# yhinai/EIG-KL-Algorithm

Measured on AMD Instinct MI355X. Metric: wall-clock to final cut (s) + cut size, ibm18.hgr; SpMV GB/s vs HBM peak, lower is better.
Workload: dtype f64 (Lanczos) + f32 (KL gains, bit-exact with cKL)

## Files before the change

eig-kl-algorithm_amd/csrc/ctx_lanczos.cpp:

```cpp
#include "ctx.hpp"

#ifndef EK_UPD_RED_MAX_NRB
#define EK_UPD_RED_MAX_NRB 256
#endif

using namespace ek::rt;

extern "C" {

void ek_lanczos_default_opts(ek_lanczos_opts* o) {
    if (!o) return;
    o->ncv = 0;
    o->maxit = 1000;
    o->tol = 1e-10;
    o->deflate = 1;
    o->time_spmv = 0;
    o->reorth = 3;
    o->check_every = 8;
    o->basis32 = 1;
    o->alpha_last = 0;
    o->keep_min = -1;
    o->reorth_thresh = 0.0;
}

// ... 236 lines not shown
        ek::dev::ProLaunch pl;
        if (inl) {
            pl.wpart = c->wpart.as<double>();
            pl.alpha = c->alpha.as<double>();
            pl.offd = c->offd.as<double>();
            pl.omega = c->omega.as<double>();
            pl.st = c->prost.as<ek::dev::ProState>();
            pl.flags = c->pflags.as<int>();
            pl.pub = pro_pub();
            pl.a3 = a3;
            pl.seg0 = seg0;
            pl.m = m;
            pl.thresh = pro_thresh;
            pl.eps1 = pro_eps1;
            pl.cgw = pro_cgw;
            static const int tickets = env_flag("EK_PRO_TICKETS", false) ? 2 : env_flag("EK_PRO_TICKETS", true) ? 1 : 0;
            if (tickets) pl.tix = pro_pub() + size_t(ek::dev::PRO_PUB_WORDS) * ek::dev::PRO_PUB_STRIDE;
            if (tickets == 1) {
                pl.cap = ek::dev::gemvt_pro_capacity(nt, c->nrb_spmv > 12 * 256, pro_merge, pro_merge && b32,
                                                     c->num_cu);
                const int ncg_max = (m + has_u0 + ek::dev::GT_COLS - 1) / ek::dev::GT_COLS;
                auto grid = [&](int cg) { return ek::dev::gemvt_pro_grid(nrb, std::min(ncg_max, cg), ldv, pro_merge); };
                int cg = pl.cgw;
                while (!pro_cgw_env && cg > 1 && grid(cg) > pl.cap) --cg;
                if (!pro_cgw_env && cg > 0 && grid(cg) <= pl.cap) pl.cgw = cg;
            }
            pl.rev = env_set("EK_DISPATCH_REVERSE") ? 1 : 0;
            if (pro_merge) {
                pl.merged = 1;
                pl.npart = c->npart.as<double>();
                pl.V32 = V32();
                pl.fb = b32 ? c->fbk.as<unsigned>() : nullptr;
            }
        }
        const bool mrg = inl && pro_merge;
        for (int i = k; i < kend; ++i) {
            ek::dev::StepFin fin;
            if (i > seg0) {
                fin.npart = c->npart.as<double>();
                fin.nb = nub;
                fin.fn2_out = fn2 + i;
                fin.h2 = c->h2.as<double>();
                fin.step = i - 1;
                fin.alpha = c->alpha.as<double>();
                fin.offd = c->offd.as<double>();
                fin.a3 = a3;
                fin.fn2_i = fn2 + i - 1;
                fin.bov_i = bov + i - 1;
// ... 902 lines not shown
```

eig-kl-algorithm_amd/csrc/ek_internal.hpp:

```cpp
#pragma once

#include <cstdint>
#include <cstdio>
#include <cstring>
#include <functional>
#include <memory>
#include <utility>
#include <string>
#include <type_traits>
#include <vector>

#include "../../include/eigkl.h"

namespace ek {
void set_error(const char* fmt, ...) __attribute__((format(printf, 1, 2)));
struct Error {
    int code;
};
[[noreturn]] void fail(int code, const char* fmt, ...) __attribute__((format(printf, 2, 3)));
int guard_exceptions();

int host_threads();
struct ThreadCap {
    explicit ThreadCap(int cap);
// ... 317 lines not shown
              int i, int seg0, int m, double thresh, double eps1);
constexpr int PRO_PUB = 8;
constexpr int PRO_PUB_STRIDE = 64;
constexpr int PRO_PUB_WORDS = PRO_PUB + 1;
struct ProLaunch {
    const double* wpart = nullptr;
    const double* alpha = nullptr;
    const double* offd = nullptr;
    double* omega = nullptr;
    ProState* st = nullptr;
    int* flags = nullptr;
    unsigned* pub = nullptr;
    double* a3 = nullptr;
    double* npart = nullptr;
    const float* V32 = nullptr;
    unsigned* fb = nullptr;
    int merged = 0;
    int cgw = 0;
    int seg0 = 0, m = 0;
    double thresh = 0.0, eps1 = 0.0;
    unsigned* tix = nullptr;
    int rev = 0;
    int cap = 0;
};
int gemvt_pro_capacity(bool nt, bool wide, bool merged, bool b32u, int num_cu);
int gemvt_pro_grid(int nrb, int ncgl, int ldv, bool merged);
void finalize_step(hipStream_t s, const double* npart, int nb, double* fn2_out, const double* h1,
                   const double* h2, int step, double* alpha, double* offd, const double* a3 = nullptr,
                   const double* fn2_i = nullptr, const double* bov_i = nullptr);
void three_term(hipStream_t s, int ldv, const double* apart, int nparts, double* alpha_io, const double* w,
                const double* vi, const double* vim1, const double* fn2_i, const double* bov_i, double* fp,
                float* v32col = nullptr);
void gemm_vq(hipStream_t s, int ldv, const double* V, int m, const double* Q, int kk, double* out,
             float* out32 = nullptr);
void inject_random(hipStream_t s, double* f, int ldv, long long row0, long long nrows, unsigned long long st0);
void zero_pad_rows(hipStream_t s, double* V, int ldv, int nreal, int ncols);
size_t split_tmp_bytes(int n);
void fiedler_scale(hipStream_t s, const double* x, double sgn, int n, double* out);
void split_select(hipStream_t s, void* tmp, const double* v, int n, unsigned k0, unsigned k1,
                  unsigned long long* keys_out);
double key_value(unsigned long long key);
void split_partition(hipStream_t s, void* tmp, const double* v, int n, double med, int32_t* order0, int32_t* order1,
                     uint32_t* plist, uint8_t* side, unsigned* n0_out);
void axpby_norm(hipStream_t s, int ldv, double* f, double sigma, const double* x, double hk, double* npart);
void scale_sub_mean(hipStream_t s, int ldv, double* x, int nreal, const double* mean_sum, double inv_n);
void sum_partial(hipStream_t s, int ldv, const double* x, int nreal, double* npart, int squares);
void resid_partial(hipStream_t s, int ldv, const double* w, const double* x, double lambda, int nreal, double* part);
void start_vector(hipStream_t s, int ldv, long long row0, int nreal, double* x);

// ... 195 lines not shown
```

eig-kl-algorithm_amd/csrc/kernels_lanczos.hip:

```cpp
#include <hip/hip_runtime.h>

#include <cstdio>
#include <cstdlib>

#include "ek_device.hpp"
#include "ek_internal.hpp"

#ifndef EK_UPD_UB
#define EK_UPD_UB 8
#endif

namespace ek {
namespace dev {

#ifdef EK_PRO_STAMPS
constexpr int PRO_STAMP_LO = 20, PRO_STAMP_NS = 80, PRO_STAMP_WG = 2048, PRO_STAMP_W = 6;
__device__ unsigned long long g_pro_stamps[size_t(PRO_STAMP_NS) * PRO_STAMP_WG * PRO_STAMP_W];
__device__ __forceinline__ void pro_stamp(int step, int slot, unsigned long long val) {
    const int k = step - PRO_STAMP_LO;
    if (threadIdx.x == 0 && k >= 0 && k < PRO_STAMP_NS && int(blockIdx.x) < PRO_STAMP_WG)
        g_pro_stamps[(size_t(k) * PRO_STAMP_WG + blockIdx.x) * PRO_STAMP_W + slot] = val;
}
#define PRO_STAMP(slot) pro_stamp(ncols - 1, (slot), __builtin_amdgcn_s_memrealtime())
#define PRO_ROLE(r) pro_stamp(ncols - 1, 0, (r))
#define PRO_DECISION(v) pro_stamp(ncols - 1, 5, (v))
#else
#define PRO_STAMP(slot) ((void)0)
#define PRO_ROLE(r) ((void)0)
#define PRO_DECISION(v) ((void)0)
#endif

#ifndef EK_PRO_CG0_FIRST
#define EK_PRO_CG0_FIRST 1
#endif
#ifndef EK_PRO_NORM_DIRECT
#define EK_PRO_NORM_DIRECT 1
#endif
__host__ __device__ constexpr int pro_slots(int nrb) { return EK_PRO_CG0_FIRST ? (nrb + 7) / 8 * 8 : nrb; }

__device__ __forceinline__ double wave_sum(double v) {
#pragma unroll
    for (int o = 32; o > 0; o >>= 1) v += __shfl_xor(v, o, 64);
    return v;
}

__device__ __forceinline__ double strided_sum256(const double* __restrict__ x, int n) {
    constexpr int SB = 16;
    double s = 0.0;
    if (n <= 0) return s;
    for (int i0 = threadIdx.x; i0 < n; i0 += SB * 256) {
        double v[SB];
#pragma unroll
        for (int u = 0; u < SB; ++u) v[u] = x[min(i0 + u * 256, n - 1)];
#pragma unroll
        for (int u = 0; u < SB; ++u) s += i0 + u * 256 < n ? v[u] : 0.0;
    }
    return s;
}

__device__ __forceinline__ void strided_sum256x2(const double* __restrict__ x, const double* __restrict__ y, int n,
                                                 double& sx, double& sy) {
// ... 149 lines not shown
    __syncthreads();
    double mx = fabs(nv);
#pragma unroll
    for (int o = 32; o > 0; o >>= 1) mx = fmax(mx, __shfl_xor(mx, o, 64));
    if ((t & 63) == 0) mx4[t >> 6] = mx;
    __syncthreads();
    const double mxa = fmax(fmax(mx4[0], mx4[1]), fmax(mx4[2], mx4[3]));
    const bool d = forced || !(mxa <= thresh);
    if (t < i) onew[t] = d ? eps1 : nv;
    if (t == i) onew[i] = eps1;
    if (t == 255) onew[U] = d ? eps1 : nv;
    if (i == seg0) {
        if (t < i) ocur[t] = eps1;
        if (t == 255) ocur[U] = eps1;
    }
    if (t == 0) {
        flags[i] = d ? 1 : 0;
        st->force = (d && !s_pair) ? 1 : 0;
        if (d) st->projected += 1;
    }
    return d;
}

__device__ __forceinline__ void gemvt_skip_tail(int ncols, int has_u0, int nrb, int rbk, int t,
                                                double* __restrict__ part, const double* nred,
                                                unsigned* __restrict__ gctr, double* __restrict__ h_out,
                                                double* __restrict__ fn2_fast, bool zero_h = true,
                                                unsigned* __restrict__ done = nullptr) {
    const int tot = ncols + has_u0, i = ncols - 1;
    __syncthreads();
    const double nb = (nred[0] + nred[1]) + (nred[2] + nred[3]);
    if (!h_out) {
        if (t == 0) part[size_t(tot) * nrb + rbk] = nb;
        if (t == 1) part[size_t(i) * nrb + rbk] = 0.0;
        if (t == 2 && i > 0) part[size_t(i - 1) * nrb + rbk] = 0.0;
        return;
    }
    __shared__ int s_last;
    if (t == 0) {
        st_sc1(part + size_t(tot) * nrb + rbk, nb);
        asm volatile("s_waitcnt vmcnt(0)" ::: "memory");
        const int g = rbk % GT_SUB;
        const unsigned gsize = unsigned((nrb - g + GT_SUB - 1) / GT_SUB), ngroups = unsigned(nrb < GT_SUB ? nrb : GT_SUB);
        int last = 0;
        if (__hip_atomic_fetch_add(gctr + g * 64, 1u, EK_HANDOFF_ORDER, __HIP_MEMORY_SCOPE_AGENT) == gsize - 1u)
            last = __hip_atomic_fetch_add(gctr + GT_SUB * 64, 1u, EK_HANDOFF_ORDER, __HIP_MEMORY_SCOPE_AGENT) ==
                   ngroups - 1u;
        s_last = last;
    }
    __syncthreads();
    if (!s_last) return;
    if (zero_h)
        for (int j = t; j < tot; j += 256) h_out[j] = 0.0;
    if (t < CS_LANES) {
        const double* pc = part + size_t(tot) * nrb;
        constexpr int CB = 32;
        double a = 0.0;
        for (int b0 = t; b0 < nrb; b0 += CS_LANES * CB) {
            double va[CB];
#pragma unroll
            for (int u = 0; u < CB; ++u) va[u] = ld_sc1(pc + min(b0 + CS_LANES * u, nrb - 1));
#pragma unroll
            for (int u = 0; u < CB; ++u) a += b0 + CS_LANES * u < nrb ? va[u] : 0.0;
        }
#pragma unroll
        for (int o = 1; o < CS_LANES; o <<= 1) a += __shfl_xor(a, o, 64);
        if (t == 0) {
            if (done) {
                st_sc1(h_out + tot, a);
                if (fn2_fast) st_sc1(fn2_fast, a);
                asm volatile("s_waitcnt vmcnt(0)" ::: "memory");
                __hip_atomic_fetch_add(done, 1u, __ATOMIC_RELAXED, __HIP_MEMORY_SCOPE_AGENT);
            } else {
                h_out[tot] = a;
                if (fn2_fast) *fn2_fast = a;
            }
        }
    }
    if (t < GT_SUB + 1) gctr[t * 64] = 0u;
}

__device__ __forceinline__ bool pro_aborted(int* err) {
    return __hip_atomic_load(err, __ATOMIC_RELAXED, __HIP_MEMORY_SCOPE_AGENT) != 0;
}
__device__ __forceinline__ int pro_poll(const unsigned* pub, int* err) {
    unsigned v = 0u;
    for (int it = 0; it < (1 << 22); ++it) {
        v = __hip_atomic_load(pub, __ATOMIC_RELAXED, __HIP_MEMORY_SCOPE_AGENT);
        if (v != 0u) break;
        if ((it & 255) == 255 && pro_aborted(err)) break;
        __builtin_amdgcn_s_sleep(8);
    }
    if (v == 0u) atomicAdd(err, 1);
    return v != 0u ? int(v) : 2;
}
__device__ __forceinline__ int pro_wait(const unsigned* ctr, unsigned target, int* err) {
    for (int it = 0; it < (1 << 22); ++it) {
        if (__hip_atomic_load(ctr, __ATOMIC_RELAXED, __HIP_MEMORY_SCOPE_AGENT) >= target) return 1;
        if ((it & 255) == 255 && pro_aborted(err)) break;
        __builtin_amdgcn_s_sleep(4);
    }
    atomicAdd(err, 1);
    return 0;
}

struct UpdTT {
    const double* w = nullptr;
    const double* vi = nullptr;
    const double* vim1 = nullptr;
    const double* fn2_i = nullptr;
    const double* bov_i = nullptr;
    const double* apart = nullptr;
    int nparts = 0;
    int* err = nullptr;
};
template <bool RED, bool B32, bool NT, bool MRG>
__device__ __forceinline__ void update_body(int blk, int ldv, const double* __restrict__ V, int ncols, int has_u0,
                                            double u0val, int nreal, const double* __restrict__ h,
                                            const double* __restrict__ src, double* __restrict__ dst,
                                            double* __restrict__ npart, const double* __restrict__ part, int nrb,
                                            double* __restrict__ h_out, const float* __restrict__ V32,
                                            unsigned* __restrict__ fb, double* __restrict__ fn2_fast,
                                            const unsigned* __restrict__ done, unsigned done_target, UpdTT tt);

template <bool TT, bool NT, int APE, bool PROI, bool MRG = false, bool B32U = false>
__device__ __forceinline__ void gemvt_body(int ldv, int nrb, const double* __restrict__ V, int ncols,
                                               int has_u0, double u0val, int nreal, const double* __restrict__ w,
                                               double* __restrict__ part, const double* __restrict__ alpha,
                                               const double* __restrict__ vi, const double* __restrict__ vim1,
                                               const double* __restrict__ fn2_i, const double* __restrict__ bov_i,
                                               double* __restrict__ fp, int nrm, float* __restrict__ v32col,
                                               const double* __restrict__ apart, int nparts,
                                               double* __restrict__ alpha_pub, unsigned* __restrict__ gctr,
                                               double* __restrict__ h_out, const int* __restrict__ flag,
                                               double* __restrict__ fn2_fast, ProLaunch pl) {
#pragma clang fp contract(off)
    __shared__ double red[4][GT_COLS];
    __shared__ double nred[4];
    __shared__ double lds4[4];
    __shared__ double s_alpha;
    const int t = threadIdx.x;
    const int ncg = (ncols + has_u0 + GT_COLS - 1) / GT_COLS;
    const int ncgl = PROI && pl.cgw > 0 ? min(ncg, pl.cgw) : ncg;
    int nwg = int(gridDim.x), orig = int(blockIdx.x);
    if constexpr (PROI) {
        if (pl.rev) orig = nwg - 1 - orig;
        if (pl.tix) {
            __shared__ int s_orig;
            if (t == 0) {
                const unsigned x = unsigned(orig) & 7u, cnt = (unsigned(nwg) - x + 7u) >> 3;
                unsigned* q = pl.tix + PRO_PUB_STRIDE * x;
                const unsigned j = __hip_atomic_fetch_add(q, 1u, __ATOMIC_RELAXED, __HIP_MEMORY_SCOPE_AGENT);
                if (j == cnt - 1u) __hip_atomic_store(q, 0u, __ATOMIC_RELAXED, __HIP_MEMORY_SCOPE_AGENT);
                s_orig = int(x + 8u * j);
            }
            __syncthreads();
            orig = s_orig;
        }
    }
    if constexpr (PROI) PRO_STAMP(1);
    if constexpr (PROI) {
        if (orig < 8) {
            PRO_ROLE(orig == 0 ? 1 : 2);
            if (orig == 0) {
                const bool d = pro_decide(apart, pl.wpart, nparts, pl.a3, fn2_i, bov_i, pl.alpha, pl.offd, pl.omega,
                                          pl.st, pl.flags, ncols - 1, pl.seg0, pl.m, pl.thresh, pl.eps1);
                if (t < PRO_PUB)
                    __hip_atomic_store(pl.pub + PRO_PUB_STRIDE * t, d ? 2u : 1u, __ATOMIC_RELAXED,
                                       __HIP_MEMORY_SCOPE_AGENT);
                PRO_STAMP(2);
                PRO_DECISION(d ? 2 : 1);
            }
            PRO_STAMP(4);
            return;
        }
        orig -= 8;
        nwg -= 8;
        if constexpr (MRG) {
            const int nproj = pro_slots(nrb) * ncgl;
            if (orig >= nproj) {
                const int blk = orig - nproj, tot = ncols + has_u0;
                unsigned* done = pl.pub + PRO_PUB_STRIDE * PRO_PUB;
                __shared__ int s_ud;
                PRO_ROLE(5);
                if (t == 0) s_ud = pro_poll(pl.pub + PRO_PUB_STRIDE * (orig % 8), &pl.st->timeouts);
                PRO_STAMP(2);
                __syncthreads();
                if (s_ud == 1) {
                    if (blk == 0) {
                        if (t == 0 && !(B32U && EK_PRO_NORM_DIRECT)) {
                            (void)pro_wait(done, 1u, &pl.st->timeouts);
                            PRO_STAMP(3);
                            if (fn2_fast) *fn2_fast = ld_sc1(h_out + tot);
                        }
                        if (t < 2 && ncols - 1 - t >= 0) h_out[ncols - 1 - t] = 0.0;
                    }
                    PRO_STAMP(4);
                    return;
                }
                UpdTT tt;
                tt.w = w;
                tt.vi = vi;
                tt.vim1 = vim1;
                tt.fn2_i = fn2_i;
                tt.bov_i = bov_i;
                tt.apart = apart;
                tt.nparts = nparts;
                tt.err = &pl.st->timeouts;
                update_body<false, B32U, NT, true>(blk, ldv, V, ncols, has_u0, u0val, nreal, h_out, fp, fp, pl.npart,
                                                   nullptr, nrb, nullptr, pl.V32, pl.fb, fn2_fast, done,
                                                   unsigned(ncg + 1), tt);
                PRO_STAMP(4);
                return;
            }
            nwg = nproj;
        }
    }
    int xcd = orig % 8;
    const int q = nwg / 8, rr = nwg % 8;
    bool skip = !PROI && flag && *flag == 0;
    if (skip && orig >= nrb) return;
    int rbk, j0;
    if (PROI && EK_PRO_CG0_FIRST) {
        const int P1 = pro_slots(nrb), ph = orig / P1, o = orig % P1, idx = o / 8;
        xcd = o % 8;
        const int b8 = nrb / 8, e8 = nrb % 8;
        if (idx >= b8 + (xcd < e8 ? 1 : 0)) return;
        rbk = xcd * b8 + min(xcd, e8) + idx;
        j0 = ph * GT_COLS;
    } else {
        const int v = skip ? orig * ncgl : (xcd < rr ? xcd * (q + 1) : rr * (q + 1) + (xcd - rr) * q) + orig / 8;
        rbk = v / ncgl;
        j0 = (v % ncgl) * GT_COLS;
    }
    __shared__ int s_dec;
    if constexpr (PROI) {
        PRO_ROLE(j0 == 0 ? 3 : 4);
        if (j0 != 0) {
            if (t == 0) s_dec = pro_poll(pl.pub + PRO_PUB_STRIDE * xcd, &pl.st->timeouts);
            PRO_STAMP(2);
            __syncthreads();
            if (s_dec == 1) {
                PRO_STAMP(4);
                return;
            }
        }
    }
    const bool v_first = !PROI && !skip;
    double acc[GT_COLS];
#pragma unroll
    for (int jj = 0; jj < GT_COLS; ++jj) acc[jj] = 0.0;
// ... 47 lines not shown
            y.y = __builtin_fma(-a, tv[k].y, y.y);
            if (vim1) {
                y.x = __builtin_fma(-b, tu[k].x, y.x);
                y.y = __builtin_fma(-b, tu[k].y, y.y);
            }
            xs[k] = y;
            if (j0 == 0) {
                const size_t r = size_t(rbk) * GT_ROWS + size_t(k) * 512 + 2 * size_t(t);
                if constexpr (!MRG) out_store2(fp + r, y);
                if (v32col) *reinterpret_cast<float2*>(v32col + r) = make_float2(float(tv[k].x), float(tv[k].y));
            }
        }
    }
    if (nrm && j0 == 0) {
        double s = 0.0;
#pragma unroll
        for (int k = 0; k < KR; ++k) s += __builtin_fma(xs[k].x, xs[k].x, xs[k].y * xs[k].y);
        s = wave_sum(s);
        if ((t & 63) == 0) nred[t >> 6] = s;
    }
    if constexpr (PROI) {
        if (j0 == 0) {
            PRO_STAMP(2);
            gemvt_skip_tail(ncols, has_u0, nrb, rbk, t, part, nred, gctr + GT_NORM_CTR, h_out,
                            MRG && !(B32U && EK_PRO_NORM_DIRECT) ? nullptr : fn2_fast, false,
                            MRG ? pl.pub + PRO_PUB_STRIDE * PRO_PUB : nullptr);
            PRO_STAMP(3);
            if (t == 0) s_dec = pro_poll(pl.pub + PRO_PUB_STRIDE * xcd, &pl.st->timeouts);
            __syncthreads();
            skip = s_dec == 1;
            if constexpr (MRG) {
                if (skip) {
#pragma unroll
                    for (int k = 0; k < KR; ++k)
                        out_store2(fp + size_t(rbk) * GT_ROWS + size_t(k) * 512 + 2 * size_t(t), xs[k]);
                }
            }
            if (skip) {
                PRO_STAMP(4);
                return;
            }
        }
    }
    if (skip) {
        gemvt_skip_tail(ncols, has_u0, nrb, rbk, t, part, nred, gctr, h_out, fn2_fast);
        return;
    }
    const int jstep = ncgl * GT_COLS, jend = PROI ? ncg * GT_COLS : j0 + 1;
    for (int jc = j0; jc < jend; jc += jstep) {
    if (PROI) {
        if (jc != j0) {
            __syncthreads();
#pragma unroll
            for (int jj = 0; jj < GT_COLS; ++jj) acc[jj] = 0.0;
        }
#pragma unroll
        for (int k = 0; k < KR; ++k) {
            const size_t r = size_t(rbk) * GT_ROWS + size_t(k) * 512 + 2 * size_t(t);
// ... 27 lines not shown
    {
        const bool hi = lane & 16;
#pragma unroll
        for (int k = 0; k < 2; ++k) a2[k] = (hi ? a4[k + 2] : a4[k]) + __shfl_xor(hi ? a4[k] : a4[k + 2], 16, 64);
    }
    double a1;
    {
        const bool hi = lane & 8;
        a1 = (hi ? a2[1] : a2[0]) + __shfl_xor(hi ? a2[0] : a2[1], 8, 64);
    }
    a1 += __shfl_xor(a1, 4, 64);
    a1 += __shfl_xor(a1, 2, 64);
    a1 += __shfl_xor(a1, 1, 64);
    if ((lane & 7) == 0) red[t >> 6][((lane >> 5) & 1) * 4 + ((lane >> 4) & 1) * 2 + ((lane >> 3) & 1)] = a1;
    __syncthreads();
    const int tot = ncols + has_u0;
    if (!h_out) {
        if (t < GT_COLS && jc + t < tot) part[size_t(jc + t) * nrb + rbk] = (red[0][t] + red[1][t]) + (red[2][t] + red[3][t]);
        if (nrm && jc == 0 && t == 0) part[size_t(tot) * nrb + rbk] = (nred[0] + nred[1]) + (nred[2] + nred[3]);
        continue;
    }
    __shared__ int s_last;
    if (t < GT_COLS && jc + t < tot) st_sc1(part + size_t(jc + t) * nrb + rbk, (red[0][t] + red[1][t]) + (red[2][t] + red[3][t]));
    if (!PROI && nrm && jc == 0 && t == 0) st_sc1(part + size_t(tot) * nrb + rbk, (nred[0] + nred[1]) + (nred[2] + nred[3]));
    const int cg = jc / GT_COLS;
    unsigned* ctr = gctr + size_t(cg) * (GT_SUB + 1) * 64;
    if (t == 0) {
        asm volatile("s_waitcnt vmcnt(0)" ::: "memory");
        const int g = rbk % GT_SUB;
        const unsigned gsize = unsigned((nrb - g + GT_SUB - 1) / GT_SUB), ngroups = unsigned(nrb < GT_SUB ? nrb : GT_SUB);
        int last = 0;
        if (__hip_atomic_fetch_add(ctr + g * 64, 1u, EK_HANDOFF_ORDER, __HIP_MEMORY_SCOPE_AGENT) == gsize - 1u)
            last = __hip_atomic_fetch_add(ctr + GT_SUB * 64, 1u, EK_HANDOFF_ORDER, __HIP_MEMORY_SCOPE_AGENT) ==
                   ngroups - 1u;
        s_last = last;
    }
    __syncthreads();
    if (!s_last) continue;
    const int gq = t / CS_LANES, l = t % CS_LANES;
    const int ncol = min(GT_COLS, tot - jc) + ((nrm && jc == 0 && !PROI) ? 1 : 0);
    if (gq < ncol) {
        const int j = gq < GT_COLS && jc + gq < tot ? jc + gq : tot;
        const double* pc = part + size_t(j) * nrb;
        constexpr int CB = 32;
        double a = 0.0;
        for (int b0 = l; b0 < nrb; b0 += CS_LANES * CB) {
            double va[CB];
#pragma unroll
            for (int u = 0; u < CB; ++u) va[u] = ld_sc1(pc + min(b0 + CS_LANES * u, nrb - 1));
#pragma unroll
            for (int u = 0; u < CB; ++u) a += b0 + CS_LANES * u < nrb ? va[u] : 0.0;
        }
#pragma unroll
        for (int o = 1; o < CS_LANES; o <<= 1) a += __shfl_xor(a, o, 64);
        if (l == 0) {
            if constexpr (MRG) st_sc1(h_out + j, a);
            else h_out[j] = a;
        }
    }
    if constexpr (MRG) {
        asm volatile("s_waitcnt vmcnt(0)" ::: "memory");
        __syncthreads();
        if (t == 0)
            __hip_atomic_fetch_add(pl.pub + PRO_PUB_STRIDE * PRO_PUB, 1u, __ATOMIC_RELAXED, __HIP_MEMORY_SCOPE_AGENT);
    }
    if (t < GT_SUB + 1) ctr[t * 64] = 0u;
    }
    if constexpr (PROI) PRO_STAMP(4);
}

#define EK_GEMVT_PARAMS                                                                                               \
    int ldv, int nrb, const double *__restrict__ V, int ncols, int has_u0, double u0val, int nreal,                  \
        const double *__restrict__ w, double *__restrict__ part, const double *__restrict__ alpha,                   \
        const double *__restrict__ vi, const double *__restrict__ vim1, const double *__restrict__ fn2_i,            \
        const double *__restrict__ bov_i, double *__restrict__ fp, int nrm, float *__restrict__ v32col,              \
        const double *__restrict__ apart, int nparts, double *__restrict__ alpha_pub, unsigned *__restrict__ gctr,   \
        double *__restrict__ h_out, const int *__restrict__ flag, double *__restrict__ fn2_fast, ProLaunch pl
#define EK_GEMVT_ARGS                                                                                                \
    ldv, nrb, V, ncols, has_u0, u0val, nreal, w, part, alpha, vi, vim1, fn2_i, bov_i, fp, nrm, v32col, apart, nparts,  \
        alpha_pub, gctr, h_out, flag, fn2_fast, pl
template <bool TT, bool NT, int APE = 12>
__global__ __launch_bounds__(256) void k_gemvt(EK_GEMVT_PARAMS) {
    gemvt_body<TT, NT, APE, false>(EK_GEMVT_ARGS);
}
template <bool NT, int APE, bool MRG, bool B32U>
__global__ __launch_bounds__(256) __attribute__((amdgpu_waves_per_eu(4))) void k_gemvt_pro(EK_GEMVT_PARAMS) {
    gemvt_body<true, NT, APE, true, MRG, B32U>(EK_GEMVT_ARGS);
}
#undef EK_GEMVT_PARAMS
#undef EK_GEMVT_ARGS

__global__ __launch_bounds__(256) void k_gemvt3(int ldv, int nrb, const double* __restrict__ V, int ncols,
                                                int has_u0, double u0val, int nreal, const double* __restrict__ w,
                                                const double* __restrict__ va, const double* __restrict__ vb,
                                                double* __restrict__ part) {
    __shared__ double red[3][4][GT_COLS];
    __shared__ double nred[4];
    const int t = threadIdx.x;
    const int tot = ncols + has_u0;
    const int ncg = (tot + GT_COLS - 1) / GT_COLS;
    const int nwg = int(gridDim.x), orig = int(blockIdx.x), xcd = orig % 8, q = nwg / 8, rr = nwg % 8;
    const int v = (xcd < rr ? xcd * (q + 1) : rr * (q + 1) + (xcd - rr) * q) + orig / 8;
    const int rbk = v / ncg, j0 = (v % ncg) * GT_COLS;
    const size_t nr = size_t(nreal);
    constexpr int KR = GT_ROWS / 512;
    const int jmax = ncols > 0 ? ncols - 1 : 0;
    double2 xs[3][KR], vs[KR][GT_COLS];
#pragma unroll
    for (int k = 0; k < KR; ++k) {
        const size_t r = size_t(rbk) * GT_ROWS + size_t(k) * 512 + 2 * size_t(t);
// ... 119 lines not shown
#pragma unroll
            for (int u = 0; u < PT; ++u)
                if (t + 256 * u < cn) st[q * RC_LD + t + 256 * u] = v[q][u];
        __syncthreads();
        if (g < RC_COLS) {
            const double* col = st + g * RC_LD;
            int i = l;
            for (; i + 3 * CS_LANES < cn; i += 4 * CS_LANES) {
                const double x0 = col[i], x1 = col[i + CS_LANES], x2 = col[i + 2 * CS_LANES], x3 = col[i + 3 * CS_LANES];
                a += x0;
                a += x1;
                a += x2;
                a += x3;
            }
            for (; i < cn; i += CS_LANES) a += col[i];
        }
        __syncthreads();
    }
#pragma unroll
    for (int o = 1; o < CS_LANES; o <<= 1) a += __shfl_xor(a, o, 64);
    if (g < RC_COLS && l == 0 && j0 + g < ncols) h[j0 + g] = a;
}

template <bool RED, bool B32, bool NT, bool MRG>
__device__ __forceinline__ void update_body(int blk, int ldv, const double* __restrict__ V, int ncols, int has_u0,
                                            double u0val, int nreal, const double* __restrict__ h,
                                            const double* __restrict__ src, double* __restrict__ dst,
                                            double* __restrict__ npart, const double* __restrict__ part, int nrb,
                                            double* __restrict__ h_out, const float* __restrict__ V32,
                                            unsigned* __restrict__ fb, double* __restrict__ fn2_fast,
                                            const unsigned* __restrict__ done, unsigned done_target, UpdTT tt) {
#pragma clang fp contract(off)
    if constexpr (!B32) {
        if (fn2_fast && blk == 0 && threadIdx.x == 0) *fn2_fast = __builtin_nan("");
    }
    constexpr int UB = EK_UPD_UB;
    constexpr int UB32 = 2 * EK_UPD_UB;
    constexpr int UBX = B32 ? UB32 : UB;
    __shared__ double hc[MAX_NCV + 2 * UBX];
    __shared__ double hu0, snrm;
    __shared__ double lds4[4];
    const int tot = ncols + has_u0;
    const int totr = tot + (B32 ? 1 : 0);
    const int jmax = ncols > 0 ? ncols - 1 : 0;
    const size_t r = (size_t(blk) * 256 + threadIdx.x) * 2;
    auto load_batch = [&](double2* vb, int j0) {
#pragma unroll
        for (int u = 0; u < UB; ++u) vb[u] = ld_basis<NT>(V + size_t(min(j0 + u, jmax)) * ldv + r);
    };
    double2 x = make_double2(0.0, 0.0);
    if constexpr (!MRG) {
        x = *reinterpret_cast<const double2*>(src + r);
    } else {
        const double2 ttw = *reinterpret_cast<const double2*>(tt.w + r);
        const double2 ttv = *reinterpret_cast<const double2*>(tt.vi + r);
        const double2 ttu = tt.vim1 ? *reinterpret_cast<const double2*>(tt.vim1 + r) : make_double2(0.0, 0.0);
        __shared__ double s_al;
        const double sa = block_sum256(strided_sum256(tt.apart, tt.nparts), lds4);
        if (threadIdx.x == 0) s_al = sa;
        __syncthreads();
        const double a = s_al;
        const double b = tt.vim1 ? (isnan(*tt.bov_i) ? sqrt(*tt.fn2_i) : *tt.bov_i) : 0.0;
        x = ttw;
        x.x = __builtin_fma(-a, ttv.x, x.x);
        x.y = __builtin_fma(-a, ttv.y, x.y);
        if (tt.vim1) {
            x.x = __builtin_fma(-b, ttu.x, x.x);
            x.y = __builtin_fma(-b, ttu.y, x.y);
        }
    }
    auto consume = [&](const double2* vb, int j0) {
#pragma unroll
        for (int u = 0; u < UB; ++u) {
            const double hj = hc[j0 + u];
            x.x = __builtin_fma(-vb[u].x, hj, x.x);
// ... 406 lines not shown
}

__global__ __launch_bounds__(256) void k_sub_mean(double* __restrict__ x, int nreal, const double* __restrict__ sum,
                                                  double inv_n) {
    const size_t r = size_t(blockIdx.x) * 256 + threadIdx.x;
    if (r < size_t(nreal)) x[r] -= (*sum) * inv_n;
}

void gemvt(hipStream_t s, int ldv, int nrb, const double* V, int ncols, int has_u0, double u0val, int nreal,
           const double* w, double* part, int nrm, unsigned* gctr, double* h_out, bool nt) {
    const int cols = ncols + has_u0;
    if (cols <= 0) return;
    const dim3 g(nrb * ((cols + GT_COLS - 1) / GT_COLS));
    if (nt)
        hipLaunchKernelGGL((k_gemvt<false, true>), g, dim3(256), 0, s, ldv, nrb, V, ncols, has_u0, u0val, nreal, w, part,
                           nullptr, nullptr, nullptr, nullptr, nullptr, nullptr, nrm, nullptr, nullptr, 0, nullptr, gctr,
                           h_out, nullptr, nullptr, ProLaunch{});
    else
        hipLaunchKernelGGL((k_gemvt<false, false>), g, dim3(256), 0, s, ldv, nrb, V, ncols, has_u0, u0val, nreal, w, part,
                           nullptr, nullptr, nullptr, nullptr, nullptr, nullptr, nrm, nullptr, nullptr, 0, nullptr, gctr,
                           h_out, nullptr, nullptr, ProLaunch{});
}

int gemvt_pro_grid(int nrb, int ncgl, int ldv, bool merged) {
    return (EK_PRO_CG0_FIRST ? pro_slots(nrb) : nrb) * ncgl + 8 + (merged ? ldv / UPD_ROWS : 0);
}

int gemvt_pro_capacity(bool nt, bool wide, bool merged, bool b32u, int num_cu) {
    int per = 0;
#define EK_PRO_OCC(NT_, APE_, M_, B_)                                                                         \
    (void)hipOccupancyMaxActiveBlocksPerMultiprocessor(&per, reinterpret_cast<const void*>(&k_gemvt_pro<NT_, APE_, M_, B_>), \
                                                       256, 0)
#define EK_PRO_OCC_NT(APE_)                                     \
    do {                                                        \
        if (nt) {                                               \
            if (!merged) EK_PRO_OCC(true, APE_, false, false);  \
            else if (b32u) EK_PRO_OCC(true, APE_, true, true);  \
            else EK_PRO_OCC(true, APE_, true, false);           \
        } else {                                                \
            if (!merged) EK_PRO_OCC(false, APE_, false, false); \
            else if (b32u) EK_PRO_OCC(false, APE_, true, true); \
            else EK_PRO_OCC(false, APE_, true, false);          \
        }                                                       \
    } while (0)
    if (wide) EK_PRO_OCC_NT(24);
    else EK_PRO_OCC_NT(12);
#undef EK_PRO_OCC_NT
#undef EK_PRO_OCC
    return per * num_cu;
}

void gemvt_tt(hipStream_t s, int ldv, int nrb, const double* V, int ncols, int has_u0, double u0val, int nreal,
              const double* w, const double* alpha, const double* vi, const double* vim1, const double* fn2_i,
              const double* bov_i, double* fp, double* part, float* v32col, const double* apart, int nparts,
              unsigned* gctr, double* h_out, bool nt, const int* flag, double* fn2_fast, const ProLaunch* pl) {
    const int cols = ncols + has_u0;
    const bool mrg = pl && pl->merged;
    const int ncg = (cols + GT_COLS - 1) / GT_COLS, ncgl = pl && pl->cgw > 0 ? std::min(ncg, pl->cgw) : ncg;
    const dim3 g((pl && EK_PRO_CG0_FIRST ? pro_slots(nrb) : nrb) * ncgl + (pl ? 8 : 0) + (mrg ? ldv / UPD_ROWS : 0));
    ProLaunch pv = pl ? *pl : ProLaunch{};
    if (pv.tix && pv.cap > 0 && int(g.x) <= pv.cap) pv.tix = nullptr;
#define EK_GEMVT_TT(KERNEL_)                                                                                           \
    hipLaunchKernelGGL(KERNEL_, g, dim3(256), 0, s, ldv, nrb, V, ncols, has_u0, u0val, nreal,                         \
                       w, part, apart ? nullptr : alpha, vi, vim1, fn2_i, bov_i, fp, (v32col || flag || pl) ? 1 : 0,   \
                       v32col, apart, nparts, apart ? const_cast<double*>(alpha) : nullptr, gctr, h_out, flag,       \
                       fn2_fast, pv)
    const bool wide = apart && nparts > 12 * 256;
    if (pl) {
        if (!apart || !pl->pub || !gctr || !h_out) {
            std::fprintf(stderr, "gemvt_tt: the in-launch decision needs the alpha partials and the hand-off\n");
            std::abort();
        }
#define EK_GEMVT_PRO(NT_, APE_)                                                      \
    do {                                                                            \
        if (!mrg) EK_GEMVT_TT((k_gemvt_pro<NT_, APE_, false, false>));              \
        else if (pl->V32) EK_GEMVT_TT((k_gemvt_pro<NT_, APE_, true, true>));        \
        else EK_GEMVT_TT((k_gemvt_pro<NT_, APE_, true, false>));                    \
    } while (0)
        if (nt) {
            if (wide) EK_GEMVT_PRO(true, 24);
            else EK_GEMVT_PRO(true, 12);
        } else {
            if (wide) EK_GEMVT_PRO(false, 24);
            else EK_GEMVT_PRO(false, 12);
        }
#undef EK_GEMVT_PRO
    } else if (nt) {
        if (wide) EK_GEMVT_TT((k_gemvt<true, true, 24>));
        else EK_GEMVT_TT((k_gemvt<true, true, 12>));
    } else {
        if (wide) EK_GEMVT_TT((k_gemvt<true, false, 24>));
        else EK_GEMVT_TT((k_gemvt<true, false, 12>));
    }
#undef EK_GEMVT_TT
}


void gemvt3(hipStream_t s, int ldv, int nrb, const double* V, int ncols, int has_u0, double u0val, int nreal,
            const double* w, const double* va, const double* vb, double* part) {
// ... 189 lines not shown
    }
    x[r] = v;
}

void start_vector(hipStream_t s, int ldv, long long row0, int nreal, double* x) {
    hipLaunchKernelGGL(k_start_vector, dim3((ldv + 255) / 256), dim3(256), 0, s, x, ldv, row0, nreal);
}

void resid_partial(hipStream_t s, int ldv, const double* w, const double* x, double lambda, int nreal, double* part) {
    hipLaunchKernelGGL(k_resid_partial, dim3(ldv / UPD_ROWS), dim3(256), 0, s, w, x, lambda, nreal, part);
}

void sum_partial(hipStream_t s, int ldv, const double* x, int nreal, double* npart, int squares) {
    hipLaunchKernelGGL(k_sum_partial, dim3(ldv / UPD_ROWS), dim3(256), 0, s, x, nreal, npart, squares);
}

void scale_sub_mean(hipStream_t s, int ldv, double* x, int nreal, const double* mean_sum, double inv_n) {
    hipLaunchKernelGGL(k_sub_mean, dim3(ldv / 256), dim3(256), 0, s, x, nreal, mean_sum, inv_n);
}

}
}

#ifdef EK_PRO_STAMPS
extern "C" int ek_lab_pro_stamps(unsigned long long* out, long long count) {
    const long long cap = (long long)(sizeof(ek::dev::g_pro_stamps) / sizeof(unsigned long long));
    if (count > cap) count = cap;
    return hipMemcpyFromSymbol(out, HIP_SYMBOL(ek::dev::g_pro_stamps), size_t(count) * 8, 0, hipMemcpyDeviceToHost) ==
                   hipSuccess
               ? int(count)
               : -1;
}
#endif
```

include/eigkl.h:

```cpp
#ifndef EIGKL_H
#define EIGKL_H

#include <stdint.h>

#ifdef __cplusplus
extern "C" {
#endif

enum ek_status {
    EK_OK = 0,
    EK_EINVAL = -1,
    EK_EIO = -2,
    EK_EHIP = -3,
    EK_ENOMEM = -4,
    EK_ENOCONV = -5,
    EK_ESTATE = -6,
    EK_ECOMM = -7
};

const char* ek_last_error(void);
const char* ek_version(void);
#define EIGKL_ABI_VERSION 4
int ek_abi_version(void);

// ... 73 lines not shown
} ek_lanczos_opts;

typedef struct {
    int32_t restarts;
    int32_t matvecs;
    int32_t converged;
    double residual;
    double total_ms;
    double spmv_ms;
    int32_t spmv_timed;
    double comm_ms;
    int32_t allgathers;
    int32_t allreduces;
    int32_t update32_steps;
    int32_t update32_fallbacks;
    int32_t projected_steps;
    int32_t reprojected;
    double ortho_max;
} ek_lanczos_stats;

void ek_lanczos_default_opts(ek_lanczos_opts* o);
int ek_lanczos_fiedler(ek_ctx* ctx, const ek_lanczos_opts* o, double* lambda_out, double* v_host_out,
                       ek_lanczos_stats* stats);

int ek_median_split(int64_t n, const double* v, double* median_out, uint8_t* bits_out);
int ek_align_sign(int64_t n, double* v, const double* ref);
int ek_eig_write(const char* path, int64_t n, double lambda, double median, const uint8_t* bits,
                 const double* v);
int ek_eig_read(const char* path, int64_t n, double* lambda, double* median, uint8_t* bits, double* v,
                int32_t* order0, int64_t* n0, int32_t* order1, int64_t* n1);

typedef struct {
    uint32_t iter;
    uint32_t node_left;
    uint32_t node_right;
    float max_gain, min_gain;
    float gain;
    float cut;
    uint32_t pad;
} ek_swap;

typedef struct {
    int64_t iterations;
    float initial_cut, best_cut, final_cut;
    int64_t best_iter;
    int64_t net_cut_initial, net_cut_best, net_cut_final;
// ... 248 lines not shown
```

Measured before the change: 0.05893.

## Add resident merged GEMV-T/update launch that reuses tile rows for the update

Adds a resident form of the merged projection+update Lanczos kernel. Projection workgroups no longer hand off to separately scheduled update blocks; each one performs handoff arrival for its strided column groups and then runs the vector update on its own row tile, passing the already-loaded x values in directly. This removes the extra update workgroups and the ticket dispatch, and avoids reloading w/v to rebuild x. In exchange it requires the whole grid to fit within occupancy capacity, aborting otherwise, and serialises the update behind each block's handoffs.

```diff
diff --git a/eig-kl-algorithm_amd/csrc/ctx_lanczos.cpp b/eig-kl-algorithm_amd/csrc/ctx_lanczos.cpp
--- a/eig-kl-algorithm_amd/csrc/ctx_lanczos.cpp
+++ b/eig-kl-algorithm_amd/csrc/ctx_lanczos.cpp
@@ -282,8 +282,20 @@
                 const int ncg_max = (m + has_u0 + ek::dev::GT_COLS - 1) / ek::dev::GT_COLS;
                 auto grid = [&](int cg) { return ek::dev::gemvt_pro_grid(nrb, std::min(ncg_max, cg), ldv, pro_merge); };
                 int cg = pl.cgw;
-                while (!pro_cgw_env && cg > 1 && grid(cg) > pl.cap) --cg;
-                if (!pro_cgw_env && cg > 0 && grid(cg) <= pl.cap) pl.cgw = cg;
+                if (pro_merge && !pro_cgw_env && cg > 0) {
+                    const int cap = ek::dev::gemvt_pro_capacity(nt, c->nrb_spmv > 12 * 256, true, b32, c->num_cu, true);
+                    auto rgrid = [&](int g) { return ek::dev::gemvt_pro_grid(nrb, std::min(ncg_max, g), ldv, true, true); };
+                    int rc = cg;
+                    while (rc > 1 && rgrid(rc) > cap) --rc;
+                    if (rgrid(rc) <= cap) {
+                        pl.res = 1;
+                        pl.cgw = rc;
+                        pl.cap = cap;
+                        pl.tix = nullptr;
+                    }
+                }
+                while (!pl.res && !pro_cgw_env && cg > 1 && grid(cg) > pl.cap) --cg;
+                if (!pl.res && !pro_cgw_env && cg > 0 && grid(cg) <= pl.cap) pl.cgw = cg;
             }
             pl.rev = env_set("EK_DISPATCH_REVERSE") ? 1 : 0;
             if (pro_merge) {
diff --git a/eig-kl-algorithm_amd/csrc/ek_internal.hpp b/eig-kl-algorithm_amd/csrc/ek_internal.hpp
--- a/eig-kl-algorithm_amd/csrc/ek_internal.hpp
+++ b/eig-kl-algorithm_amd/csrc/ek_internal.hpp
@@ -363,9 +363,10 @@
     unsigned* tix = nullptr;
     int rev = 0;
     int cap = 0;
-};
-int gemvt_pro_capacity(bool nt, bool wide, bool merged, bool b32u, int num_cu);
-int gemvt_pro_grid(int nrb, int ncgl, int ldv, bool merged);
+    int res = 0;
+};
+int gemvt_pro_capacity(bool nt, bool wide, bool merged, bool b32u, int num_cu, bool res = false);
+int gemvt_pro_grid(int nrb, int ncgl, int ldv, bool merged, bool res = false);
 void finalize_step(hipStream_t s, const double* npart, int nb, double* fn2_out, const double* h1,
                    const double* h2, int step, double* alpha, double* offd, const double* a3 = nullptr,
                    const double* fn2_i = nullptr, const double* bov_i = nullptr);
diff --git a/eig-kl-algorithm_amd/csrc/kernels_lanczos.hip b/eig-kl-algorithm_amd/csrc/kernels_lanczos.hip
--- a/eig-kl-algorithm_amd/csrc/kernels_lanczos.hip
+++ b/eig-kl-algorithm_amd/csrc/kernels_lanczos.hip
@@ -37,6 +37,15 @@
 #define EK_PRO_NORM_DIRECT 1
 #endif
 __host__ __device__ constexpr int pro_slots(int nrb) { return EK_PRO_CG0_FIRST ? (nrb + 7) / 8 * 8 : nrb; }
+__host__ __device__ constexpr int pro_unit0(int ph, int ncgl) { return ncgl - 1 - ph; }
+__host__ __device__ constexpr bool pro_row_block(int orig, int nrb, int* rbk, int* ph, int* xcd) {
+    const int P1 = pro_slots(nrb), o = orig % P1, idx = o / 8, x = o % 8;
+    const int b8 = nrb / 8, e8 = nrb % 8;
+    *ph = orig / P1;
+    *xcd = x;
+    *rbk = x * b8 + (x < e8 ? x : e8) + idx;
+    return idx < b8 + (x < e8 ? 1 : 0);
+}
 
 __device__ __forceinline__ double wave_sum(double v) {
 #pragma unroll
@@ -232,7 +241,28 @@
     return d;
 }
 
-__device__ __forceinline__ void gemvt_skip_tail(int ncols, int has_u0, int nrb, int rbk, int t,
+__device__ __forceinline__ double handoff_col_sum(const double* pc, int nrb, int l) {
+    constexpr int CB = 32;
+    double a = 0.0;
+    for (int b0 = l; b0 < nrb; b0 += CS_LANES * CB) {
+        double va[CB];
+#pragma unroll
+        for (int u = 0; u < CB; ++u) va[u] = ld_sc1(pc + min(b0 + CS_LANES * u, nrb - 1));
+#pragma unroll
+        for (int u = 0; u < CB; ++u) a += b0 + CS_LANES * u < nrb ? va[u] : 0.0;
+    }
+#pragma unroll
+    for (int o = 1; o < CS_LANES; o <<= 1) a += __shfl_xor(a, o, 64);
+    return a;
+}
+__device__ __forceinline__ bool handoff_arrive(unsigned* ctr, int nrb, int rbk) {
+    const int g = rbk % GT_SUB;
+    const unsigned gsize = unsigned((nrb - g + GT_SUB - 1) / GT_SUB), ngroups = unsigned(nrb < GT_SUB ? nrb : GT_SUB);
+    if (__hip_atomic_fetch_add(ctr + g * 64, 1u, EK_HANDOFF_ORDER, __HIP_MEMORY_SCOPE_AGENT) != gsize - 1u) return false;
+    return __hip_atomic_fetch_add(ctr + GT_SUB * 64, 1u, EK_HANDOFF_ORDER, __HIP_MEMORY_SCOPE_AGENT) == ngroups - 1u;
+}
+
+__device__ __forceinline__ bool gemvt_skip_tail(int ncols, int has_u0, int nrb, int rbk, int t,
                                                 double* __restrict__ part, const double* nred,
                                                 unsigned* __restrict__ gctr, double* __restrict__ h_out,
                                                 double* __restrict__ fn2_fast, bool zero_h = true,
@@ -244,37 +274,20 @@
         if (t == 0) part[size_t(tot) * nrb + rbk] = nb;
         if (t == 1) part[size_t(i) * nrb + rbk] = 0.0;
         if (t == 2 && i > 0) part[size_t(i - 1) * nrb + rbk] = 0.0;
-        return;
+        return false;
     }
     __shared__ int s_last;
     if (t == 0) {
         st_sc1(part + size_t(tot) * nrb + rbk, nb);
         asm volatile("s_waitcnt vmcnt(0)" ::: "memory");
-        const int g = rbk % GT_SUB;
-        const unsigned gsize = unsigned((nrb - g + GT_SUB - 1) / GT_SUB), ngroups = unsigned(nrb < GT_SUB ? nrb : GT_SUB);
-        int last = 0;
-        if (__hip_atomic_fetch_add(gctr + g * 64, 1u, EK_HANDOFF_ORDER, __HIP_MEMORY_SCOPE_AGENT) == gsize - 1u)
-            last = __hip_atomic_fetch_add(gctr + GT_SUB * 64, 1u, EK_HANDOFF_ORDER, __HIP_MEMORY_SCOPE_AGENT) ==
-                   ngroups - 1u;
-        s_last = last;
+        s_last = handoff_arrive(gctr, nrb, rbk) ? 1 : 0;
     }
     __syncthreads();
-    if (!s_last) return;
+    if (!s_last) return false;
     if (zero_h)
         for (int j = t; j < tot; j += 256) h_out[j] = 0.0;
     if (t < CS_LANES) {
-        const double* pc = part + size_t(tot) * nrb;
-        constexpr int CB = 32;
-        double a = 0.0;
-        for (int b0 = t; b0 < nrb; b0 += CS_LANES * CB) {
-            double va[CB];
-#pragma unroll
-            for (int u = 0; u < CB; ++u) va[u] = ld_sc1(pc + min(b0 + CS_LANES * u, nrb - 1));
-#pragma unroll
-            for (int u = 0; u < CB; ++u) a += b0 + CS_LANES * u < nrb ? va[u] : 0.0;
-        }
-#pragma unroll
-        for (int o = 1; o < CS_LANES; o <<= 1) a += __shfl_xor(a, o, 64);
+        const double a = handoff_col_sum(part + size_t(tot) * nrb, nrb, t);
         if (t == 0) {
             if (done) {
                 st_sc1(h_out + tot, a);
@@ -288,6 +301,7 @@
         }
     }
     if (t < GT_SUB + 1) gctr[t * 64] = 0u;
+    return true;
 }
 
 __device__ __forceinline__ bool pro_aborted(int* err) {
@@ -323,8 +337,9 @@
     const double* apart = nullptr;
     int nparts = 0;
     int* err = nullptr;
+    double2 x = {0.0, 0.0};
 };
-template <bool RED, bool B32, bool NT, bool MRG>
+template <bool RED, bool B32, bool NT, bool MRG, bool XIN = false>
 __device__ __forceinline__ void update_body(int blk, int ldv, const double* __restrict__ V, int ncols, int has_u0,
                                             double u0val, int nreal, const double* __restrict__ h,
                                             const double* __restrict__ src, double* __restrict__ dst,
@@ -333,7 +348,7 @@
                                             unsigned* __restrict__ fb, double* __restrict__ fn2_fast,
                                             const unsigned* __restrict__ done, unsigned done_target, UpdTT tt);
 
-template <bool TT, bool NT, int APE, bool PROI, bool MRG = false, bool B32U = false>
+template <bool TT, bool NT, int APE, bool PROI, bool MRG = false, bool B32U = false, bool RES = false>
 __device__ __forceinline__ void gemvt_body(int ldv, int nrb, const double* __restrict__ V, int ncols,
                                                int has_u0, double u0val, int nreal, const double* __restrict__ w,
                                                double* __restrict__ part, const double* __restrict__ alpha,
@@ -354,8 +369,9 @@
     const int ncgl = PROI && pl.cgw > 0 ? min(ncg, pl.cgw) : ncg;
     int nwg = int(gridDim.x), orig = int(blockIdx.x);
     if constexpr (PROI) {
+        static_assert(!RES || (MRG && EK_PRO_CG0_FIRST), "the resident form is the merged launch's");
         if (pl.rev) orig = nwg - 1 - orig;
-        if (pl.tix) {
+        if (!RES && pl.tix) {
             __shared__ int s_orig;
             if (t == 0) {
                 const unsigned x = unsigned(orig) & 7u, cnt = (unsigned(nwg) - x + 7u) >> 3;
@@ -386,7 +402,7 @@
         }
         orig -= 8;
         nwg -= 8;
-        if constexpr (MRG) {
+        if constexpr (MRG && !RES) {
             const int nproj = pro_slots(nrb) * ncgl;
             if (orig >= nproj) {
                 const int blk = orig - nproj, tot = ncols + has_u0;
@@ -432,11 +448,8 @@
     if (skip && orig >= nrb) return;
     int rbk, j0;
     if (PROI && EK_PRO_CG0_FIRST) {
-        const int P1 = pro_slots(nrb), ph = orig / P1, o = orig % P1, idx = o / 8;
-        xcd = o % 8;
-        const int b8 = nrb / 8, e8 = nrb % 8;
-        if (idx >= b8 + (xcd < e8 ? 1 : 0)) return;
-        rbk = xcd * b8 + min(xcd, e8) + idx;
+        int ph;
+        if (!pro_row_block(orig, nrb, &rbk, &ph, &xcd)) return;
         j0 = ph * GT_COLS;
     } else {
         const int v = skip ? orig * ncgl : (xcd < rr ? xcd * (q + 1) : rr * (q + 1) + (xcd - rr) * q) + orig / 8;
@@ -530,9 +543,10 @@
     if constexpr (PROI) {
         if (j0 == 0) {
             PRO_STAMP(2);
-            gemvt_skip_tail(ncols, has_u0, nrb, rbk, t, part, nred, gctr + GT_NORM_CTR, h_out,
-                            MRG && !(B32U && EK_PRO_NORM_DIRECT) ? nullptr : fn2_fast, false,
-                            MRG ? pl.pub + PRO_PUB_STRIDE * PRO_PUB : nullptr);
+            const bool norm_last =
+                gemvt_skip_tail(ncols, has_u0, nrb, rbk, t, part, nred, gctr + GT_NORM_CTR, h_out,
+                                MRG && !(B32U && EK_PRO_NORM_DIRECT) ? nullptr : fn2_fast, false,
+                                MRG ? pl.pub + PRO_PUB_STRIDE * PRO_PUB : nullptr);
             PRO_STAMP(3);
             if (t == 0) s_dec = pro_poll(pl.pub + PRO_PUB_STRIDE * xcd, &pl.st->timeouts);
             __syncthreads();
@@ -542,6 +556,13 @@
 #pragma unroll
                     for (int k = 0; k < KR; ++k)
                         out_store2(fp + size_t(rbk) * GT_ROWS + size_t(k) * 512 + 2 * size_t(t), xs[k]);
+                }
+            }
+            if constexpr (RES) {
+                if (skip && norm_last) {
+                    if (t == 0 && !(B32U && EK_PRO_NORM_DIRECT) && fn2_fast)
+                        *fn2_fast = ld_sc1(h_out + ncols + has_u0);
+                    if (t < 2 && ncols - 1 - t >= 0) h_out[ncols - 1 - t] = 0.0;
                 }
             }
             if (skip) {
@@ -615,18 +636,13 @@
     }
     __shared__ int s_last;
     if (t < GT_COLS && jc + t < tot) st_sc1(part + size_t(jc + t) * nrb + rbk, (red[0][t] + red[1][t]) + (red[2][t] + red[3][t]));
+    if constexpr (RES) continue;
     if (!PROI && nrm && jc == 0 && t == 0) st_sc1(part + size_t(tot) * nrb + rbk, (nred[0] + nred[1]) + (nred[2] + nred[3]));
     const int cg = jc / GT_COLS;
     unsigned* ctr = gctr + size_t(cg) * (GT_SUB + 1) * 64;
     if (t == 0) {
         asm volatile("s_waitcnt vmcnt(0)" ::: "memory");
-        const int g = rbk % GT_SUB;
-        const unsigned gsize = unsigned((nrb - g + GT_SUB - 1) / GT_SUB), ngroups = unsigned(nrb < GT_SUB ? nrb : GT_SUB);
-        int last = 0;
-        if (__hip_atomic_fetch_add(ctr + g * 64, 1u, EK_HANDOFF_ORDER, __HIP_MEMORY_SCOPE_AGENT) == gsize - 1u)
-            last = __hip_atomic_fetch_add(ctr + GT_SUB * 64, 1u, EK_HANDOFF_ORDER, __HIP_MEMORY_SCOPE_AGENT) ==
-                   ngroups - 1u;
-        s_last = last;
+        s_last = handoff_arrive(ctr, nrb, rbk) ? 1 : 0;
     }
     __syncthreads();
     if (!s_last) continue;
@@ -634,18 +650,7 @@
     const int ncol = min(GT_COLS, tot - jc) + ((nrm && jc == 0 && !PROI) ? 1 : 0);
     if (gq < ncol) {
         const int j = gq < GT_COLS && jc + gq < tot ? jc + gq : tot;
-        const double* pc = part + size_t(j) * nrb;
-        constexpr int CB = 32;
-        double a = 0.0;
-        for (int b0 = l; b0 < nrb; b0 += CS_LANES * CB) {
-            double va[CB];
-#pragma unroll
-            for (int u = 0; u < CB; ++u) va[u] = ld_sc1(pc + min(b0 + CS_LANES * u, nrb - 1));
-#pragma unroll
-            for (int u = 0; u < CB; ++u) a += b0 + CS_LANES * u < nrb ? va[u] : 0.0;
-        }
-#pragma unroll
-        for (int o = 1; o < CS_LANES; o <<= 1) a += __shfl_xor(a, o, 64);
+        const double a = handoff_col_sum(part + size_t(j) * nrb, nrb, l);
         if (l == 0) {
             if constexpr (MRG) st_sc1(h_out + j, a);
             else h_out[j] = a;
@@ -658,6 +663,43 @@
             __hip_atomic_fetch_add(pl.pub + PRO_PUB_STRIDE * PRO_PUB, 1u, __ATOMIC_RELAXED, __HIP_MEMORY_SCOPE_AGENT);
     }
     if (t < GT_SUB + 1) ctr[t * 64] = 0u;
+    }
+    if constexpr (RES) {
+        const int tot = ncols + has_u0, ph = j0 / GT_COLS;
+        unsigned* done = pl.pub + PRO_PUB_STRIDE * PRO_PUB;
+        if (t < 64) {
+            asm volatile("s_waitcnt vmcnt(0)" ::: "memory");
+            const int cgk = ph + t * ncgl;
+            bool last = false;
+            if (cgk < ncg) last = handoff_arrive(gctr + size_t(cgk) * (GT_SUB + 1) * 64, nrb, rbk);
+            for (unsigned long long mask = __ballot(last); mask; mask &= mask - 1) {
+                const int cg = ph + __builtin_ctzll(mask) * ncgl, jc = cg * GT_COLS;
+                unsigned* ctr = gctr + size_t(cg) * (GT_SUB + 1) * 64;
+                const int gq = t / CS_LANES, l = t % CS_LANES;
+                if (gq < min(GT_COLS, tot - jc)) {
+                    const double a = handoff_col_sum(part + size_t(jc + gq) * nrb, nrb, l);
+                    if (l == 0) st_sc1(h_out + jc + gq, a);
+                }
+                asm volatile("s_waitcnt vmcnt(0)" ::: "memory");
+                if (t == 0) __hip_atomic_fetch_add(done, 1u, __ATOMIC_RELAXED, __HIP_MEMORY_SCOPE_AGENT);
+                if (t < GT_SUB + 1) ctr[t * 64] = 0u;
+            }
+        }
+        PRO_STAMP(3);
+        constexpr int NU = GT_ROWS / UPD_ROWS;
+        static_assert(NU == KR && UPD_ROWS == 512, "an update unit is one k of the tile's rows");
+        for (int u = pro_unit0(ph, ncgl); u < NU; u += ncgl) {
+            UpdTT tt;
+            tt.err = &pl.st->timeouts;
+            tt.x = xs[0];
+#pragma unroll
+            for (int k = 1; k < KR; ++k)
+                if (u == k) tt.x = xs[k];
+            update_body<false, B32U, NT, true, true>(rbk * NU + u, ldv, V, ncols, has_u0, u0val, nreal, h_out, fp, fp,
+                                                     pl.npart, nullptr, nrb, nullptr, pl.V32, pl.fb, fn2_fast, done,
+                                                     unsigned(ncg + 1), tt);
+            __syncthreads();
+        }
     }
     if constexpr (PROI) PRO_STAMP(4);
 }
@@ -676,9 +718,9 @@
 __global__ __launch_bounds__(256) void k_gemvt(EK_GEMVT_PARAMS) {
     gemvt_body<TT, NT, APE, false>(EK_GEMVT_ARGS);
 }
-template <bool NT, int APE, bool MRG, bool B32U>
+template <bool NT, int APE, bool MRG, bool B32U, bool RES = false>
 __global__ __launch_bounds__(256) __attribute__((amdgpu_waves_per_eu(4))) void k_gemvt_pro(EK_GEMVT_PARAMS) {
-    gemvt_body<true, NT, APE, true, MRG, B32U>(EK_GEMVT_ARGS);
+    gemvt_body<true, NT, APE, true, MRG, B32U, RES>(EK_GEMVT_ARGS);
 }
 #undef EK_GEMVT_PARAMS
 #undef EK_GEMVT_ARGS
@@ -844,7 +886,7 @@
     if (g < RC_COLS && l == 0 && j0 + g < ncols) h[j0 + g] = a;
 }
 
-template <bool RED, bool B32, bool NT, bool MRG>
+template <bool RED, bool B32, bool NT, bool MRG, bool XIN>
 __device__ __forceinline__ void update_body(int blk, int ldv, const double* __restrict__ V, int ncols, int has_u0,
                                             double u0val, int nreal, const double* __restrict__ h,
                                             const double* __restrict__ src, double* __restrict__ dst,
@@ -873,6 +915,8 @@
     double2 x = make_double2(0.0, 0.0);
     if constexpr (!MRG) {
         x = *reinterpret_cast<const double2*>(src + r);
+    } else if constexpr (XIN) {
+        x = tt.x;
     } else {
         const double2 ttw = *reinterpret_cast<const double2*>(tt.w + r);
         const double2 ttv = *reinterpret_cast<const double2*>(tt.vi + r);
@@ -1325,30 +1369,32 @@
                            h_out, nullptr, nullptr, ProLaunch{});
 }
 
-int gemvt_pro_grid(int nrb, int ncgl, int ldv, bool merged) {
-    return (EK_PRO_CG0_FIRST ? pro_slots(nrb) : nrb) * ncgl + 8 + (merged ? ldv / UPD_ROWS : 0);
-}
-
-int gemvt_pro_capacity(bool nt, bool wide, bool merged, bool b32u, int num_cu) {
+int gemvt_pro_grid(int nrb, int ncgl, int ldv, bool merged, bool res) {
+    return (EK_PRO_CG0_FIRST ? pro_slots(nrb) : nrb) * ncgl + 8 + (merged && !res ? ldv / UPD_ROWS : 0);
+}
+
+int gemvt_pro_capacity(bool nt, bool wide, bool merged, bool b32u, int num_cu, bool res) {
     int per = 0;
-#define EK_PRO_OCC(NT_, APE_, M_, B_)                                                                         \
-    (void)hipOccupancyMaxActiveBlocksPerMultiprocessor(&per, reinterpret_cast<const void*>(&k_gemvt_pro<NT_, APE_, M_, B_>), \
-                                                       256, 0)
-#define EK_PRO_OCC_NT(APE_)                                     \
-    do {                                                        \
-        if (nt) {                                               \
-            if (!merged) EK_PRO_OCC(true, APE_, false, false);  \
-            else if (b32u) EK_PRO_OCC(true, APE_, true, true);  \
-            else EK_PRO_OCC(true, APE_, true, false);           \
-        } else {                                                \
-            if (!merged) EK_PRO_OCC(false, APE_, false, false); \
-            else if (b32u) EK_PRO_OCC(false, APE_, true, true); \
-            else EK_PRO_OCC(false, APE_, true, false);          \
-        }                                                       \
+#define EK_PRO_OCC(NT_, APE_, M_, B_, R_)                                                                  \
+    (void)hipOccupancyMaxActiveBlocksPerMultiprocessor(                                                    \
+        &per, reinterpret_cast<const void*>(&k_gemvt_pro<NT_, APE_, M_, B_, R_>), 256, 0)
+#define EK_PRO_OCC_M(NT_, APE_)                                         \
+    do {                                                                \
+        if (!merged) EK_PRO_OCC(NT_, APE_, false, false, false);        \
+        else if (b32u && res) EK_PRO_OCC(NT_, APE_, true, true, true);  \
+        else if (b32u) EK_PRO_OCC(NT_, APE_, true, true, false);        \
+        else if (res) EK_PRO_OCC(NT_, APE_, true, false, true);         \
+        else EK_PRO_OCC(NT_, APE_, true, false, false);                 \
+    } while (0)
+#define EK_PRO_OCC_NT(APE_)                    \
+    do {                                       \
+        if (nt) EK_PRO_OCC_M(true, APE_);      \
+        else EK_PRO_OCC_M(false, APE_);        \
     } while (0)
     if (wide) EK_PRO_OCC_NT(24);
     else EK_PRO_OCC_NT(12);
 #undef EK_PRO_OCC_NT
+#undef EK_PRO_OCC_M
 #undef EK_PRO_OCC
     return per * num_cu;
 }
@@ -1359,9 +1405,15 @@
               unsigned* gctr, double* h_out, bool nt, const int* flag, double* fn2_fast, const ProLaunch* pl) {
     const int cols = ncols + has_u0;
     const bool mrg = pl && pl->merged;
+    const bool res = mrg && pl->res;
     const int ncg = (cols + GT_COLS - 1) / GT_COLS, ncgl = pl && pl->cgw > 0 ? std::min(ncg, pl->cgw) : ncg;
-    const dim3 g((pl && EK_PRO_CG0_FIRST ? pro_slots(nrb) : nrb) * ncgl + (pl ? 8 : 0) + (mrg ? ldv / UPD_ROWS : 0));
+    const dim3 g((pl && EK_PRO_CG0_FIRST ? pro_slots(nrb) : nrb) * ncgl + (pl ? 8 : 0) +
+                 (mrg && !res ? ldv / UPD_ROWS : 0));
     ProLaunch pv = pl ? *pl : ProLaunch{};
+    if (res && (pv.cap <= 0 || int(g.x) > pv.cap || !EK_PRO_CG0_FIRST)) {
+        std::fprintf(stderr, "gemvt_tt: the resident launch's grid (%u) exceeds the capacity (%d)\n", g.x, pv.cap);
+        std::abort();
+    }
     if (pv.tix && pv.cap > 0 && int(g.x) <= pv.cap) pv.tix = nullptr;
 #define EK_GEMVT_TT(KERNEL_)                                                                                           \
     hipLaunchKernelGGL(KERNEL_, g, dim3(256), 0, s, ldv, nrb, V, ncols, has_u0, u0val, nreal,                         \
@@ -1377,7 +1429,9 @@
 #define EK_GEMVT_PRO(NT_, APE_)                                                      \
     do {                                                                            \
         if (!mrg) EK_GEMVT_TT((k_gemvt_pro<NT_, APE_, false, false>));              \
+        else if (pl->V32 && res) EK_GEMVT_TT((k_gemvt_pro<NT_, APE_, true, true, true>)); \
         else if (pl->V32) EK_GEMVT_TT((k_gemvt_pro<NT_, APE_, true, true>));        \
+        else if (res) EK_GEMVT_TT((k_gemvt_pro<NT_, APE_, true, false, true>));     \
         else EK_GEMVT_TT((k_gemvt_pro<NT_, APE_, true, false>));                    \
     } while (0)
         if (nt) {
@@ -1613,6 +1667,20 @@
 }
 }
 
+extern "C" int ek_lab_pro_resident_map(int nrb, int ncg, int cgw, int* tiles, int* units) {
+    using namespace ek::dev;
+    constexpr int NU = GT_ROWS / UPD_ROWS;
+    const int ncgl = cgw > 0 ? std::min(ncg, cgw) : ncg, nproj = pro_slots(nrb) * ncgl;
+    for (int orig = 0; orig < nproj; ++orig) {
+        int rbk = 0, ph = 0, xcd = 0;
+        if (!pro_row_block(orig, nrb, &rbk, &ph, &xcd)) continue;
+        if (rbk < 0 || rbk >= nrb) return -1;
+        for (int cg = ph; cg < ncg; cg += ncgl) ++tiles[size_t(rbk) * ncg + cg];
+        for (int u = pro_unit0(ph, ncgl); u < NU; u += ncgl) ++units[size_t(rbk) * NU + u];
+    }
+    return gemvt_pro_grid(nrb, ncgl, 0, true, true);
+}
+
 #ifdef EK_PRO_STAMPS
 extern "C" int ek_lab_pro_stamps(unsigned long long* out, long long count) {
     const long long cap = (long long)(sizeof(ek::dev::g_pro_stamps) / sizeof(unsigned long long));
diff --git a/include/eigkl.h b/include/eigkl.h
--- a/include/eigkl.h
+++ b/include/eigkl.h
@@ -119,6 +119,7 @@
 void ek_lanczos_default_opts(ek_lanczos_opts* o);
 int ek_lanczos_fiedler(ek_ctx* ctx, const ek_lanczos_opts* o, double* lambda_out, double* v_host_out,
                        ek_lanczos_stats* stats);
+int ek_lab_pro_resident_map(int nrb, int ncg, int cgw, int* tiles, int* units);
 
 int ek_median_split(int64_t n, const double* v, double* median_out, uint8_t* bits_out);
 int ek_align_sign(int64_t n, double* v, const double* ref);
```

After: 0.05905. No clear change (+0.2%).
